# jmoraispk/DeepMIMO

Hardware: AMD Instinct MI355X
Metric: user-channels/sec (higher is better)
Workload: dtype f16x3-split MFMA, f32 accumulate

## Files before the change

deepmimo_amd/csrc/k2c_beam_power.hip:

```cpp
#include "k2_mfma_frag.h"
#include "dmx_tuning.h"
#include <stdlib.h>

namespace dmx {

static constexpr int BP_SLOT = 16 * 1024;
static constexpr int BP_BUFS = 2;

struct BeamPowArgs {
    int64_t user_begin;
    int m_rx, ue_mh, n_beams;
    int M;
    int K;
    const int32_t* sc;
    double inv_n;
    const float2* ftab;
    const int32_t* fexp;
    float* out;
    int32_t* best;
    int adaptive;
};

__host__ __device__ inline size_t beam_pow_lds_bytes(int M, int NW) {
    const size_t nblk = ((size_t)M + 32 * NW - 1) / (32 * NW);
    return (size_t)BP_BUFS * (NW / 4) * BP_SLOT + LPAD * (8 + 4 + 4) + 16 + nblk * NW * 32 * 4;
}

template <int NW>
__global__ __launch_bounds__(NW * 64, 4) void k2c_beam_power(WsView ws, BeamPowArgs a, int64_t user_count) {
    constexpr int BP_WAVES = NW, BP_CHUNK = NW / 4, MAX_ROWS = 32 * NW;
    extern __shared__ __attribute__((aligned(16))) unsigned char smem[];
    unsigned char* bbuf = smem;
    float* bbuf_f = reinterpret_cast<float*>(smem);
    float2* qtab = reinterpret_cast<float2*>(smem + (size_t)BP_BUFS * BP_CHUNK * BP_SLOT);
    float* crtab = reinterpret_cast<float*>(qtab + LPAD);
    float* citab = crtab + LPAD;
    float* misc = citab + LPAD;
    float* rs = misc + 4;
    const int tid = threadIdx.x, lane = tid & 63;
    const int wave = __builtin_amdgcn_readfirstlane(tid >> 6);
    const int col = lane & 31, hh = lane >> 5;
    const int B = a.n_beams, M = a.M, P = ws.P;
    const int nwide = (a.K + 31) >> 5;
    const int nblk = (M + MAX_ROWS - 1) / MAX_ROWS;

    for (int64_t ul = blockIdx.x; ul < user_count; ul += gridDim.x) {
        const int64_t u = a.user_begin + ul;
        int n_act = ws.n_keep[u];
        n_act = n_act < LPAD ? n_act : LPAD;
        if (n_act == 0) {
            for (int b = tid; b < B; b += BP_WAVES * 64) a.out[(size_t)ul * B + b] = 0.f;
            if (a.best && tid == 0) a.best[ul] = -1;
            continue;
        }
        const size_t rb = (size_t)u * P;
        if (wave == 0) {
            float m = 0.f;
            if (lane < n_act) m = fmaxf(fabsf(ws.c_re[rb + lane]), fabsf(ws.c_im[rb + lane]));
            for (int off = 32; off > 0; off >>= 1) m = fmaxf(m, __shfl_xor(m, off));
            const int l0w = ((n_act - 1) >> 3) << 3;
            float a2 = 0.f;
            if (lane < n_act) a2 = fmaf(ws.c_re[rb + lane], ws.c_re[rb + lane], ws.c_im[rb + lane] * ws.c_im[rb + lane]);
            float m2 = a2, mw2 = lane >= l0w ? a2 : 0.f;
            for (int off = 32; off > 0; off >>= 1) { m2 = fmaxf(m2, __shfl_xor(m2, off)); mw2 = fmaxf(mw2, __shfl_xor(mw2, off)); }
            if (lane == 0) misc[3] = (a.adaptive && l0w >= 8 && mw2 * 4194304.0f <= m2) ? 1.f : 0.f;
            int e;
            (void)frexpf(m, &e);
            const float gs = ldexpf(1.0f, 10 - e);
            if (lane < LPAD) {
                const bool ok = lane < n_act;
                const double q = ok ? (double)ws.dn[rb + lane] * a.inv_n : 0.0;
                const double qh = rint(q * 4096.0) * (1.0 / 4096.0);
                qtab[lane] = make_float2((float)qh, (float)(q - qh));
                crtab[lane] = ok ? ws.c_re[rb + lane] * gs : 0.f;
                citab[lane] = ok ? ws.c_im[rb + lane] * gs : 0.f;
            }
            const int ea = 6 - a.fexp[ul];
            if (lane == 0) { misc[0] = ldexpf(1.0f, e - 10 - ea); misc[1] = ldexpf(1.0f, ea); misc[2] = gs; }
        }
        __syncthreads();
        const float ascale = misc[1];
        const int nfull = ((n_act + 7) >> 3) - (misc[3] != 0.f ? 1 : 0);

        for (int blk = 0; blk < nblk; ++blk) {
            const int row0 = blk * MAX_ROWS;
            const int nrows = (M - row0) < MAX_ROWS ? (M - row0) : MAX_ROWS;
            const int ntiles = (nrows + 31) >> 5;
            const int ntp = ntiles <= 1 ? 1 : (ntiles <= 2 ? 2 : (ntiles <= 4 ? 4 : 8));
            const int tile = wave & (ntp - 1), grp = wave / ntp, ngrp = BP_WAVES / ntp;
            const bool active = tile < ntiles;
            h8 Ah[4], Al[4];
#pragma unroll
            for (int s = 0; s < 4; ++s) { Ah[s] = h8{0, 0, 0, 0, 0, 0, 0, 0}; Al[s] = Ah[s]; }
            if (active) {
                const int r = row0 + (tile << 5) + col;
                const bool pok = r < M;
                const int rx = pok ? r / B : 0, bm = pok ? r - rx * B : 0;
                const double yr = (double)(rx % a.ue_mh), zr = (double)(rx / a.ue_mh);
                const float2* frow = a.ftab + ((size_t)ul * B + bm) * P;
#pragma unroll
                for (int s = 0; s < 4; ++s) {
                    if (8 * s < n_act) {
#pragma unroll
                        for (int jj = 0; jj < 4; ++jj) {
                            const int pl = 8 * s + 4 * hh + jj;
                            h2 vh = {(_Float16)0.f, (_Float16)0.f}, vl = vh;
                            if (pok && pl < n_act) {
                                float sn, cs;
                                sincos_rev(frac_rev(yr * ws.rx_y[rb + pl] + zr * ws.rx_z[rb + pl]), sn, cs);
                                const float2 f = frow[pl];
                                split2_f16((cs * f.x - sn * f.y) * ascale, (cs * f.y + sn * f.x) * ascale, vh, vl, ws.neg_one);
                            }
                            Ah[s][2 * jj] = vh[0]; Ah[s][2 * jj + 1] = vh[1];
                            Al[s][2 * jj] = vl[0]; Al[s][2 * jj + 1] = vl[1];
                        }
                    }
                }
            }
            typedef float pv2 __attribute__((ext_vector_type(2)));
            pv2 rowsum[8];
#pragma unroll
            for (int i = 0; i < 8; ++i) rowsum[i] = pv2{0.f, 0.f};

            auto generate = [&](int c0, int buf) {
                const int wsi = c0 + (wave >> 2), st = wave & 3;
                const int kidx = (wsi << 5) + col;
                const bool kok = wsi < nwide && kidx < a.K;
                const int kki = kok ? a.sc[kidx] : 0;
                const float kl = (float)(kki & 4095), kf = (float)kki;
                h8* slot = reinterpret_cast<h8*>(bbuf + (size_t)(buf * BP_CHUNK + (wave >> 2)) * BP_SLOT);
                h8 rh = h8{0, 0, 0, 0, 0, 0, 0, 0}, rl = rh, ih = rh, il = rh;
                if (kok && 8 * st < n_act) {
#pragma unroll
                    for (int jj = 0; jj < 4; ++jj) {
                        const int pl = 8 * st + 4 * hh + jj;
                        const float2 q = qtab[pl];
                        const float p1 = q.x * kl;
                        float sn, cs;
                        sincos_rev(fmaf(q.y, kf, p1 - rintf(p1)), sn, cs);
                        const float cr = crtab[pl], ci = citab[pl];
                        h2 vh, vl;
                        split2_f16(cr * cs + ci * sn, ci * cs - cr * sn, vh, vl, ws.neg_one);
                        const unsigned hb = __builtin_bit_cast(unsigned, vh), lb = __builtin_bit_cast(unsigned, vl);
                        const h2 reh = __builtin_bit_cast(h2, hb ^ 0x80000000u), rel = __builtin_bit_cast(h2, lb ^ 0x80000000u);
                        const h2 imh = __builtin_bit_cast(h2, __builtin_amdgcn_alignbit(hb, hb, 16));
                        const h2 iml = __builtin_bit_cast(h2, __builtin_amdgcn_alignbit(lb, lb, 16));
                        rh[2 * jj] = reh[0]; rh[2 * jj + 1] = reh[1]; rl[2 * jj] = rel[0]; rl[2 * jj + 1] = rel[1];
                        ih[2 * jj] = imh[0]; ih[2 * jj + 1] = imh[1]; il[2 * jj] = iml[0]; il[2 * jj + 1] = iml[1];
                    }
                }
                slot[(4 * st + 0) * 64 + lane] = rh;
                slot[(4 * st + 1) * 64 + lane] = rl;
                slot[(4 * st + 2) * 64 + lane] = ih;
                slot[(4 * st + 3) * 64 + lane] = il;
            };
            __syncthreads();
            generate(0, 0);
            __syncthreads();
            int buf = 0;
            for (int c0 = 0; c0 < nwide; c0 += BP_CHUNK, buf ^= 1) {
                if (c0 + BP_CHUNK < nwide) generate(c0 + BP_CHUNK, buf ^ 1);
                if (active) {
                    for (int j = grp; j < BP_CHUNK && c0 + j < nwide; j += ngrp) {
                        const h8* slot = reinterpret_cast<const h8*>(bbuf + (size_t)(buf * BP_CHUNK + j) * BP_SLOT);
                        f16v are, aim;
#pragma unroll
                        for (int i = 0; i < 16; ++i) { are[i] = 0.f; aim[i] = 0.f; }
#pragma unroll
                        for (int s = 0; s < 4; ++s) {
                            if (8 * s < n_act) {
                                const h8 rh = slot[(4 * s + 0) * 64 + lane], rl = slot[(4 * s + 1) * 64 + lane];
                                const h8 ih = slot[(4 * s + 2) * 64 + lane], il = slot[(4 * s + 3) * 64 + lane];
                                are = __builtin_amdgcn_mfma_f32_32x32x16_f16(Ah[s], rh, are, 0, 0, 0);
                                aim = __builtin_amdgcn_mfma_f32_32x32x16_f16(Ah[s], ih, aim, 0, 0, 0);
                                if (s >= nfull) continue;
                                are = __builtin_amdgcn_mfma_f32_32x32x16_f16(Ah[s], rl, are, 0, 0, 0);
                                aim = __builtin_amdgcn_mfma_f32_32x32x16_f16(Ah[s], il, aim, 0, 0, 0);
                                are = __builtin_amdgcn_mfma_f32_32x32x16_f16(Al[s], rh, are, 0, 0, 0);
                                aim = __builtin_amdgcn_mfma_f32_32x32x16_f16(Al[s], ih, aim, 0, 0, 0);
                            }
                        }
                        DMX_MFMA_RESULT_GUARD2(are, aim);
#pragma unroll
                        for (int i = 0; i < 8; ++i) {
                            const pv2 re = {are[2 * i], are[2 * i + 1]}, im = {aim[2 * i], aim[2 * i + 1]};
                            const pv2 p = __builtin_elementwise_fma(re, re, im * im);
                            rowsum[i] += pv2{__builtin_amdgcn_sqrtf(p.x), __builtin_amdgcn_sqrtf(p.y)};
                        }
                    }
                }
                __syncthreads();
            }
            if (active) {
#pragma unroll
                for (int i = 0; i < 16; ++i) {
                    float v = (i & 1) ? rowsum[i >> 1].y : rowsum[i >> 1].x;
                    for (int off = 16; off > 0; off >>= 1) v += __shfl_xor(v, off);
                    if (col == 0) rs[((blk * BP_WAVES + wave) << 5) + (i & 3) + 8 * (i >> 2) + 4 * hh] = v;
                }
            }
        }
        __syncthreads();
        const float norm = misc[0] / ((float)a.m_rx * (float)a.K);
        for (int b = tid; b < B; b += BP_WAVES * 64) {
            float t = 0.f;
            for (int rx = 0; rx < a.m_rx; ++rx) {
                const int r = rx * B + b, blk = r / MAX_ROWS, w = r - blk * MAX_ROWS, tile = w >> 5;
                const int nrows = (M - blk * MAX_ROWS) < MAX_ROWS ? (M - blk * MAX_ROWS) : MAX_ROWS;
                const int ntiles = (nrows + 31) >> 5;
                const int ntp = ntiles <= 1 ? 1 : (ntiles <= 2 ? 2 : (ntiles <= 4 ? 4 : 8));
                for (int g = 0; g < BP_WAVES / ntp; ++g) t += rs[((blk * BP_WAVES + g * ntp + tile) << 5) + (w & 31)];
            }
            t *= norm;
            a.out[(size_t)ul * B + b] = t;
            bbuf_f[b] = t;
        }
        __syncthreads();
        if (a.best && tid == 0) {
            int arg = 0;
            float mx = bbuf_f[0];
            for (int b = 1; b < B; ++b) { if (bbuf_f[b] > mx) { mx = bbuf_f[b]; arg = b; } }
            a.best[ul] = arg;
        }
        __syncthreads();
    }
}

int launch_beam_power(const dmx_params& prm, const WsView& ws, int64_t user_begin, int64_t user_count,
                      const float2* codebook, int n_beams, void* beam_ws, float* out_amp, int32_t* out_best, hipStream_t stream) {
    if (user_count == 0 || n_beams == 0) return DMX_OK;
    BeamPowArgs a;
    a.user_begin = user_begin;
    a.m_rx = prm.ue_shape[0] * prm.ue_shape[1];
    a.ue_mh = prm.ue_shape[0];
    a.n_beams = n_beams;
    a.M = a.m_rx * n_beams;
    const int nw = tuning_int("DMX_BEAM_WAVES", 8) == 4 ? 4 : 8;
    const size_t smem = beam_pow_lds_bytes(a.M, nw);
    if (smem > 160 * 1024) { set_error("%d x %d (rx, beam) rows are too many for the beam-power kernel", a.m_rx, n_beams); return DMX_ERR_SHAPE; }
    BeamTabs t;
    int rc = launch_beam_project(prm, ws, user_begin, user_count, codebook, n_beams, beam_ws, stream, &t);
    if (rc) return rc;
    a.K = prm.n_selected;
    a.sc = prm.selected_subcarriers;
    a.inv_n = 1.0 / (double)prm.n_subcarriers;
    a.ftab = t.ftab;
    a.fexp = t.fexp;
    a.out = out_amp;
    a.best = out_best;
    a.adaptive = (prm.flags & DMX_FLAG_ADAPTIVE_TERMS) ? 1 : 0;
    const auto kernel = nw == 4 ? k2c_beam_power<4> : k2c_beam_power<8>;
    int64_t grid = resident_workgroups(kernel, nw * 64, smem);
    const int64_t g4 = user_count / 4;
    if (g4 > grid) grid = g4 < 4 * grid ? g4 : 4 * grid;
    if (grid > user_count) grid = user_count;
    return launch_dyn_lds(kernel, "k2c_beam_power", dim3((unsigned)grid), dim3(nw * 64), smem, smem, stream, ws, a, user_count);
}

}
```

Baseline: 6.488 million.

## Specialize MFMA strip by step count and pack short tail step into one MFMA

Replaces the runtime-guarded MFMA loop with a templated strip function picked by a wave-uniform switch on the number of 8-path steps and whether the last step is short. When the final step holds at most two paths, it packs the hi and lo f16 parts of A and B into a single fragment so that step needs one MFMA pair per component instead of three. Also swaps __shfl_xor for direct ds_bpermute and adds asm barriers to steer register allocation. The packing depends on how lanes map to the MFMA K dimension and adds more code paths and more register pressure from the switch.

```diff
diff --git a/deepmimo_amd/csrc/k2c_beam_power.hip b/deepmimo_amd/csrc/k2c_beam_power.hip
--- a/deepmimo_amd/csrc/k2c_beam_power.hip
+++ b/deepmimo_amd/csrc/k2c_beam_power.hip
@@ -26,6 +26,39 @@
     return (size_t)BP_BUFS * (NW / 4) * BP_SLOT + LPAD * (8 + 4 + 4) + 16 + nblk * NW * 32 * 4;
 }
 
+__device__ __forceinline__ float shfl_xor_of(float v, int ln, int off) {
+    return __builtin_bit_cast(float, __builtin_amdgcn_ds_bpermute((ln ^ off) << 2, __builtin_bit_cast(int, v)));
+}
+
+typedef float pv2 __attribute__((ext_vector_type(2)));
+
+
+template <int NS, bool SHORT>
+__device__ __forceinline__ void beam_tile_strip(const h8* slot, int lane, const h8 (&Ah)[4], const h8 (&Al)[4], pv2 (&rowsum)[8]) {
+    f16v are, aim;
+#pragma unroll
+    for (int i = 0; i < 16; ++i) { are[i] = 0.f; aim[i] = 0.f; }
+#pragma unroll
+    for (int s = 0; s < NS; ++s) {
+        const h8 rh = slot[(4 * s + 0) * 64 + lane], ih = slot[(4 * s + 2) * 64 + lane];
+        are = __builtin_amdgcn_mfma_f32_32x32x16_f16(Ah[s], rh, are, 0, 0, 0);
+        aim = __builtin_amdgcn_mfma_f32_32x32x16_f16(Ah[s], ih, aim, 0, 0, 0);
+        if (SHORT && s == NS - 1) continue;
+        const h8 rl = slot[(4 * s + 1) * 64 + lane], il = slot[(4 * s + 3) * 64 + lane];
+        are = __builtin_amdgcn_mfma_f32_32x32x16_f16(Ah[s], rl, are, 0, 0, 0);
+        aim = __builtin_amdgcn_mfma_f32_32x32x16_f16(Ah[s], il, aim, 0, 0, 0);
+        are = __builtin_amdgcn_mfma_f32_32x32x16_f16(Al[s], rh, are, 0, 0, 0);
+        aim = __builtin_amdgcn_mfma_f32_32x32x16_f16(Al[s], ih, aim, 0, 0, 0);
+    }
+    DMX_MFMA_RESULT_GUARD2(are, aim);
+#pragma unroll
+    for (int i = 0; i < 8; ++i) {
+        const pv2 re = {are[2 * i], are[2 * i + 1]}, im = {aim[2 * i], aim[2 * i + 1]};
+        const pv2 p = __builtin_elementwise_fma(re, re, im * im);
+        rowsum[i] += pv2{__builtin_amdgcn_sqrtf(p.x), __builtin_amdgcn_sqrtf(p.y)};
+    }
+}
+
 template <int NW>
 __global__ __launch_bounds__(NW * 64, 4) void k2c_beam_power(WsView ws, BeamPowArgs a, int64_t user_count) {
     constexpr int BP_WAVES = NW, BP_CHUNK = NW / 4, MAX_ROWS = 32 * NW;
@@ -37,8 +70,9 @@
     float* citab = crtab + LPAD;
     float* misc = citab + LPAD;
     float* rs = misc + 4;
-    const int tid = threadIdx.x, lane = tid & 63;
-    const int wave = __builtin_amdgcn_readfirstlane(tid >> 6);
+    const int lane = threadIdx.x & 63;
+    const int wave = __builtin_amdgcn_readfirstlane(threadIdx.x >> 6);
+    const int tid = (wave << 6) + lane;
     const int col = lane & 31, hh = lane >> 5;
     const int B = a.n_beams, M = a.M, P = ws.P;
     const int nwide = (a.K + 31) >> 5;
@@ -49,38 +83,47 @@
         int n_act = ws.n_keep[u];
         n_act = n_act < LPAD ? n_act : LPAD;
         if (n_act == 0) {
+#pragma clang loop vectorize(disable) unroll(disable)
             for (int b = tid; b < B; b += BP_WAVES * 64) a.out[(size_t)ul * B + b] = 0.f;
             if (a.best && tid == 0) a.best[ul] = -1;
             continue;
         }
         const size_t rb = (size_t)u * P;
         if (wave == 0) {
+            int ln = lane;
+            asm volatile("" : "+v"(ln));
+            const size_t rl = rb + ln;
             float m = 0.f;
-            if (lane < n_act) m = fmaxf(fabsf(ws.c_re[rb + lane]), fabsf(ws.c_im[rb + lane]));
-            for (int off = 32; off > 0; off >>= 1) m = fmaxf(m, __shfl_xor(m, off));
+            if (lane < n_act) m = fmaxf(fabsf(ws.c_re[rl]), fabsf(ws.c_im[rl]));
+            for (int off = 32; off > 0; off >>= 1) m = fmaxf(m, shfl_xor_of(m, ln, off));
             const int l0w = ((n_act - 1) >> 3) << 3;
             float a2 = 0.f;
-            if (lane < n_act) a2 = fmaf(ws.c_re[rb + lane], ws.c_re[rb + lane], ws.c_im[rb + lane] * ws.c_im[rb + lane]);
+            if (lane < n_act) a2 = fmaf(ws.c_re[rl], ws.c_re[rl], ws.c_im[rl] * ws.c_im[rl]);
             float m2 = a2, mw2 = lane >= l0w ? a2 : 0.f;
-            for (int off = 32; off > 0; off >>= 1) { m2 = fmaxf(m2, __shfl_xor(m2, off)); mw2 = fmaxf(mw2, __shfl_xor(mw2, off)); }
+            for (int off = 32; off > 0; off >>= 1) { m2 = fmaxf(m2, shfl_xor_of(m2, ln, off)); mw2 = fmaxf(mw2, shfl_xor_of(mw2, ln, off)); }
             if (lane == 0) misc[3] = (a.adaptive && l0w >= 8 && mw2 * 4194304.0f <= m2) ? 1.f : 0.f;
             int e;
             (void)frexpf(m, &e);
             const float gs = ldexpf(1.0f, 10 - e);
             if (lane < LPAD) {
                 const bool ok = lane < n_act;
-                const double q = ok ? (double)ws.dn[rb + lane] * a.inv_n : 0.0;
+                float dn0 = 0.f;
+                asm volatile("" : "+v"(dn0));
+                const double q = (double)(ok ? ws.dn[rl] : dn0) * a.inv_n;
                 const double qh = rint(q * 4096.0) * (1.0 / 4096.0);
-                qtab[lane] = make_float2((float)qh, (float)(q - qh));
-                crtab[lane] = ok ? ws.c_re[rb + lane] * gs : 0.f;
-                citab[lane] = ok ? ws.c_im[rb + lane] * gs : 0.f;
+                qtab[ln] = make_float2((float)qh, (float)(q - qh));
+                crtab[ln] = ok ? ws.c_re[rl] * gs : 0.f;
+                citab[ln] = ok ? ws.c_im[rl] * gs : 0.f;
             }
             const int ea = 6 - a.fexp[ul];
             if (lane == 0) { misc[0] = ldexpf(1.0f, e - 10 - ea); misc[1] = ldexpf(1.0f, ea); misc[2] = gs; }
         }
         __syncthreads();
         const float ascale = misc[1];
-        const int nfull = ((n_act + 7) >> 3) - (misc[3] != 0.f ? 1 : 0);
+        const int nsteps = (n_act + 7) >> 3, l0w = (nsteps - 1) << 3;
+        const bool pack = (n_act - l0w <= 2) && misc[3] == 0.f;
+        const int tile_kind = __builtin_amdgcn_readfirstlane(2 * nsteps + ((misc[3] != 0.f || pack) ? 1 : 0));
+        const bool packed = __builtin_amdgcn_readfirstlane(pack ? 1 : 0) != 0;
 
         for (int blk = 0; blk < nblk; ++blk) {
             const int row0 = blk * MAX_ROWS;
@@ -98,31 +141,44 @@
                 const int rx = pok ? r / B : 0, bm = pok ? r - rx * B : 0;
                 const double yr = (double)(rx % a.ue_mh), zr = (double)(rx / a.ue_mh);
                 const float2* frow = a.ftab + ((size_t)ul * B + bm) * P;
+                auto a_prime = [&](int pl, h2& vh, h2& vl) {
+                    vh = h2{(_Float16)0.f, (_Float16)0.f}; vl = vh;
+                    if (pok && pl < n_act) {
+                        float sn, cs;
+                        sincos_rev(frac_rev(yr * ws.rx_y[rb + pl] + zr * ws.rx_z[rb + pl]), sn, cs);
+                        const float2 f = frow[pl];
+                        split2_f16((cs * f.x - sn * f.y) * ascale, (cs * f.y + sn * f.x) * ascale, vh, vl, ws.neg_one);
+                    }
+                };
 #pragma unroll
                 for (int s = 0; s < 4; ++s) {
-                    if (8 * s < n_act) {
-#pragma unroll
-                        for (int jj = 0; jj < 4; ++jj) {
-                            const int pl = 8 * s + 4 * hh + jj;
-                            h2 vh = {(_Float16)0.f, (_Float16)0.f}, vl = vh;
-                            if (pok && pl < n_act) {
-                                float sn, cs;
-                                sincos_rev(frac_rev(yr * ws.rx_y[rb + pl] + zr * ws.rx_z[rb + pl]), sn, cs);
-                                const float2 f = frow[pl];
-                                split2_f16((cs * f.x - sn * f.y) * ascale, (cs * f.y + sn * f.x) * ascale, vh, vl, ws.neg_one);
-                            }
-                            Ah[s][2 * jj] = vh[0]; Ah[s][2 * jj + 1] = vh[1];
-                            Al[s][2 * jj] = vl[0]; Al[s][2 * jj + 1] = vl[1];
-                        }
-                    }
-                }
-            }
-            typedef float pv2 __attribute__((ext_vector_type(2)));
+                    if (8 * s >= n_act) continue;
+                    if (packed && s == nsteps - 1) {
+                        h2 vh[2], vl[2];
+                        a_prime(8 * s, vh[0], vl[0]);
+                        a_prime(8 * s + 1, vh[1], vl[1]);
+                        const _Float16 z = (_Float16)0.f;
+                        Ah[s] = hh ? h8{vl[0][0], vl[0][1], vl[1][0], vl[1][1], z, z, z, z}
+                                   : h8{vh[0][0], vh[0][1], vh[1][0], vh[1][1], vh[0][0], vh[0][1], vh[1][0], vh[1][1]};
+                        continue;
+                    }
+#pragma unroll
+                    for (int jj = 0; jj < 4; ++jj) {
+                        h2 vh, vl;
+                        a_prime(8 * s + 4 * hh + jj, vh, vl);
+                        Ah[s][2 * jj] = vh[0]; Ah[s][2 * jj + 1] = vh[1];
+                        Al[s][2 * jj] = vl[0]; Al[s][2 * jj + 1] = vl[1];
+                    }
+                }
+            }
             pv2 rowsum[8];
 #pragma unroll
             for (int i = 0; i < 8; ++i) rowsum[i] = pv2{0.f, 0.f};
 
             auto generate = [&](int c0, int buf) {
+                int lane = threadIdx.x & 63;
+                asm volatile("" : "+v"(lane));
+                const int col = lane & 31, hh = lane >> 5;
                 const int wsi = c0 + (wave >> 2), st = wave & 3;
                 const int kidx = (wsi << 5) + col;
                 const bool kok = wsi < nwide && kidx < a.K;
@@ -130,21 +186,38 @@
                 const float kl = (float)(kki & 4095), kf = (float)kki;
                 h8* slot = reinterpret_cast<h8*>(bbuf + (size_t)(buf * BP_CHUNK + (wave >> 2)) * BP_SLOT);
                 h8 rh = h8{0, 0, 0, 0, 0, 0, 0, 0}, rl = rh, ih = rh, il = rh;
+                auto b_prime = [&](int pl, h2& reh, h2& rel, h2& imh, h2& iml) {
+                    const float2 q = qtab[pl];
+                    const float p1 = q.x * kl;
+                    float sn, cs;
+                    sincos_rev(fmaf(q.y, kf, p1 - rintf(p1)), sn, cs);
+                    const float cr = crtab[pl], ci = citab[pl];
+                    h2 vh, vl;
+                    split2_f16(cr * cs + ci * sn, ci * cs - cr * sn, vh, vl, ws.neg_one);
+                    const unsigned hb = __builtin_bit_cast(unsigned, vh), lb = __builtin_bit_cast(unsigned, vl);
+                    reh = __builtin_bit_cast(h2, hb ^ 0x80000000u); rel = __builtin_bit_cast(h2, lb ^ 0x80000000u);
+                    imh = __builtin_bit_cast(h2, __builtin_amdgcn_alignbit(hb, hb, 16));
+                    iml = __builtin_bit_cast(h2, __builtin_amdgcn_alignbit(lb, lb, 16));
+                };
+                if (packed && st == nsteps - 1) {
+                    if (kok) {
+                        h2 reh[2], rel[2], imh[2], iml[2];
+                        b_prime(8 * st, reh[0], rel[0], imh[0], iml[0]);
+                        b_prime(8 * st + 1, reh[1], rel[1], imh[1], iml[1]);
+                        const h2 z = {(_Float16)0.f, (_Float16)0.f};
+                        const h2 r2 = hh ? z : rel[0], r3 = hh ? z : rel[1], i2 = hh ? z : iml[0], i3 = hh ? z : iml[1];
+                        rh = h8{reh[0][0], reh[0][1], reh[1][0], reh[1][1], r2[0], r2[1], r3[0], r3[1]};
+                        ih = h8{imh[0][0], imh[0][1], imh[1][0], imh[1][1], i2[0], i2[1], i3[0], i3[1]};
+                    }
+                    slot[(4 * st + 0) * 64 + lane] = rh;
+                    slot[(4 * st + 2) * 64 + lane] = ih;
+                    return;
+                }
                 if (kok && 8 * st < n_act) {
 #pragma unroll
                     for (int jj = 0; jj < 4; ++jj) {
-                        const int pl = 8 * st + 4 * hh + jj;
-                        const float2 q = qtab[pl];
-                        const float p1 = q.x * kl;
-                        float sn, cs;
-                        sincos_rev(fmaf(q.y, kf, p1 - rintf(p1)), sn, cs);
-                        const float cr = crtab[pl], ci = citab[pl];
-                        h2 vh, vl;
-                        split2_f16(cr * cs + ci * sn, ci * cs - cr * sn, vh, vl, ws.neg_one);
-                        const unsigned hb = __builtin_bit_cast(unsigned, vh), lb = __builtin_bit_cast(unsigned, vl);
-                        const h2 reh = __builtin_bit_cast(h2, hb ^ 0x80000000u), rel = __builtin_bit_cast(h2, lb ^ 0x80000000u);
-                        const h2 imh = __builtin_bit_cast(h2, __builtin_amdgcn_alignbit(hb, hb, 16));
-                        const h2 iml = __builtin_bit_cast(h2, __builtin_amdgcn_alignbit(lb, lb, 16));
+                        h2 reh, rel, imh, iml;
+                        b_prime(8 * st + 4 * hh + jj, reh, rel, imh, iml);
                         rh[2 * jj] = reh[0]; rh[2 * jj + 1] = reh[1]; rl[2 * jj] = rel[0]; rl[2 * jj + 1] = rel[1];
                         ih[2 * jj] = imh[0]; ih[2 * jj + 1] = imh[1]; il[2 * jj] = iml[0]; il[2 * jj + 1] = iml[1];
                     }
@@ -163,46 +236,36 @@
                 if (active) {
                     for (int j = grp; j < BP_CHUNK && c0 + j < nwide; j += ngrp) {
                         const h8* slot = reinterpret_cast<const h8*>(bbuf + (size_t)(buf * BP_CHUNK + j) * BP_SLOT);
-                        f16v are, aim;
-#pragma unroll
-                        for (int i = 0; i < 16; ++i) { are[i] = 0.f; aim[i] = 0.f; }
-#pragma unroll
-                        for (int s = 0; s < 4; ++s) {
-                            if (8 * s < n_act) {
-                                const h8 rh = slot[(4 * s + 0) * 64 + lane], rl = slot[(4 * s + 1) * 64 + lane];
-                                const h8 ih = slot[(4 * s + 2) * 64 + lane], il = slot[(4 * s + 3) * 64 + lane];
-                                are = __builtin_amdgcn_mfma_f32_32x32x16_f16(Ah[s], rh, are, 0, 0, 0);
-                                aim = __builtin_amdgcn_mfma_f32_32x32x16_f16(Ah[s], ih, aim, 0, 0, 0);
-                                if (s >= nfull) continue;
-                                are = __builtin_amdgcn_mfma_f32_32x32x16_f16(Ah[s], rl, are, 0, 0, 0);
-                                aim = __builtin_amdgcn_mfma_f32_32x32x16_f16(Ah[s], il, aim, 0, 0, 0);
-                                are = __builtin_amdgcn_mfma_f32_32x32x16_f16(Al[s], rh, are, 0, 0, 0);
-                                aim = __builtin_amdgcn_mfma_f32_32x32x16_f16(Al[s], ih, aim, 0, 0, 0);
-                            }
+                        switch (tile_kind) {
+                            case 2: beam_tile_strip<1, false>(slot, lane, Ah, Al, rowsum); break;
+                            case 3: beam_tile_strip<1, true>(slot, lane, Ah, Al, rowsum); break;
+                            case 4: beam_tile_strip<2, false>(slot, lane, Ah, Al, rowsum); break;
+                            case 5: beam_tile_strip<2, true>(slot, lane, Ah, Al, rowsum); break;
+                            case 6: beam_tile_strip<3, false>(slot, lane, Ah, Al, rowsum); break;
+                            case 7: beam_tile_strip<3, true>(slot, lane, Ah, Al, rowsum); break;
+                            case 8: beam_tile_strip<4, false>(slot, lane, Ah, Al, rowsum); break;
+                            default: beam_tile_strip<4, true>(slot, lane, Ah, Al, rowsum); break;
                         }
-                        DMX_MFMA_RESULT_GUARD2(are, aim);
-#pragma unroll
-                        for (int i = 0; i < 8; ++i) {
-                            const pv2 re = {are[2 * i], are[2 * i + 1]}, im = {aim[2 * i], aim[2 * i + 1]};
-                            const pv2 p = __builtin_elementwise_fma(re, re, im * im);
-                            rowsum[i] += pv2{__builtin_amdgcn_sqrtf(p.x), __builtin_amdgcn_sqrtf(p.y)};
-                        }
                     }
                 }
                 __syncthreads();
             }
             if (active) {
+                int ln = lane;
+                asm volatile("" : "+v"(ln));
 #pragma unroll
                 for (int i = 0; i < 16; ++i) {
                     float v = (i & 1) ? rowsum[i >> 1].y : rowsum[i >> 1].x;
-                    for (int off = 16; off > 0; off >>= 1) v += __shfl_xor(v, off);
+                    for (int off = 16; off > 0; off >>= 1) v += shfl_xor_of(v, ln, off);
                     if (col == 0) rs[((blk * BP_WAVES + wave) << 5) + (i & 3) + 8 * (i >> 2) + 4 * hh] = v;
                 }
             }
         }
         __syncthreads();
-        const float norm = misc[0] / ((float)a.m_rx * (float)a.K);
-        for (int b = tid; b < B; b += BP_WAVES * 64) {
+        int tu = tid, Ku = a.K;
+        asm volatile("" : "+v"(tu), "+s"(Ku));
+        const float norm = misc[0] / ((float)a.m_rx * (float)Ku);
+        for (int b = tu; b < B; b += BP_WAVES * 64) {
             float t = 0.f;
             for (int rx = 0; rx < a.m_rx; ++rx) {
                 const int r = rx * B + b, blk = r / MAX_ROWS, w = r - blk * MAX_ROWS, tile = w >> 5;
```

New measurement: 6.490 million (median of 2 runs). Within noise of the previous version (+0.0%).
